# chu-tianxiang/QuIP-for-all

Hardware: AMD Instinct MI355X
Metric: decode tokens/sec bs=1 Llama-7B E8P12 2-bit, 1xMI355X; % HBM roofline (higher is better)
Workload: dtype i8xi8->i32 (fp16 I/O); 1 GPU; Llama-2-7B E8P12 random-init, bs=1 greedy decode, 1 hipGraph replay per token, positions [5, 833) of a 2048-slot static KV cache; layers=32, hidden=4096, ffn=11008, vocab=32000, parallelism=replicas x1 (no collective on the data path)

## Files before the change

include/quip_mi355.h:

```cpp
#ifndef QUIP_MI355_H_
#define QUIP_MI355_H_

#include <stddef.h>
#include <stdint.h>

#ifdef __cplusplus
extern "C" {
#endif

#define QUIP_ABI_VERSION 9

typedef void* quip_stream_t;

enum {
  QUIP_OK = 0,
  QUIP_ERR_NULL_POINTER = -1,
  QUIP_ERR_BAD_SHAPE = -2,
  QUIP_ERR_MISALIGNED = -3,
  QUIP_ERR_LAUNCH = -4,
  QUIP_ERR_UNSUPPORTED = -5,
  QUIP_NO_RESULT = 1
};

int quip_abi_version(void);
const char* quip_strerror(int code);
// ... 242 lines not shown
  const float* sin;
  const void* grid_packed_abs;
  void* workspace;
  void* dbg;
  int32_t n_layers, max_len, dbg_layer;
  float rms_eps, attn_scale;
  int32_t codebook;
  float resid_scale;
  int32_t shape;
  const void* grid2;
} quip_block_engine_args;
int quip_block_engine_supported(int32_t hidden, int32_t heads, int32_t kv_heads, int32_t head_dim, int32_t n_ffn, int32_t K);
size_t quip_block_engine_workspace_bytes(void);
size_t quip_block_engine_layer_bytes(void);
int quip_block_engine(const quip_block_engine_args* args, quip_stream_t stream);
int quip_debug_occupy(int32_t nwg, int32_t lds_bytes, int64_t ticks, void* sink, quip_stream_t stream);
int quip_block_engine_gqa_supported(int32_t hidden, int32_t heads, int32_t kv_heads, int32_t head_dim, int32_t n_ffn, int32_t K);
size_t quip_block_engine_gqa_workspace_bytes(void);
int quip_tile_codes(const void* qidxs, void* tiled, int64_t rows, int64_t row_bytes, quip_stream_t stream);
int quip_untile_codes(const void* tiled, void* qidxs, int64_t rows, int64_t row_bytes, quip_stream_t stream);
int quip_block_engine_g8_supported(int32_t hidden, int32_t heads, int32_t kv_heads, int32_t head_dim, int32_t n_ffn, int32_t K);
size_t quip_block_engine_g8_workspace_bytes(void);

#ifdef __cplusplus
}
#endif
#endif
```

quip_for_all_amd/capi.py:

```python
import ctypes
import os

_HERE = os.path.dirname(os.path.abspath(__file__))
LIB_PATH = os.environ.get("QUIP_LIB_PATH") or os.path.join(_HERE, "lib", "libquip_mi355.so")

_c = ctypes
_P, _I32, _I64, _F = _c.c_void_p, _c.c_int32, _c.c_int64, _c.c_float

SIGNATURES = {
    "quip_abi_version": [],
    "quip_device_cu_count": [],
    "quip_hadamard_f16": [_P, _P, _I64, _I32, _F, _P],
    "quip_hadamard": [_P, _P, _I64, _I32, _F, _I32, _P],
    "quip_had_transform_f16": [_P, _P, _I64, _I32, _I32, _I32, _I32, _P, _I32, _P, _P, _P, _P, _F, _P],
    "quip_had_transform_planes": [_P, _P, _I32, _I32, _I32, _P, _I32, _P, _F, _P],
    "quip_had_transform_fused_f16": [_P, _P, _I64, _I32, _I32, _I32, _I32, _P, _I32, _P, _P, _P, _P, _F, _P, _P],
    "quip_had_transform_planes_fused": [_P, _P, _I32, _I32, _I32, _P, _I32, _P, _F, _P, _P],
    "quip_had_transform_group_f16": [_P, _I32, _I64, _I32, _I32, _I32, _P],
    "quip_had_transform_planes_group": [_P, _I32, _I32, _I32, _I32, _P],
    "quip_e8p_gemv_planes_group": [_P, _P, _P, _P, _P, _I32, _I32, _P],
    "quip_e8p_gemv_workspace_bytes": [_I32],
    "quip_e8p_gemv_planes_ws": [_P, _P, _P, _P, _I32, _I32, _P, _c.c_size_t, _P],
    "quip_e8p_gemv_planes_group_ws": [_P, _P, _P, _P, _P, _I32, _I32, _P, _c.c_size_t, _P],
    "quip_had_transform_planes_rows": [_P, _I64, _I32, _I32, _I32, _P],
# ... 12 lines not shown
    "quip_rope_attn_workspace_bytes": [_I32, _I32],
    "quip_argmax_step_f16": [_P, _I32, _P, _P, _P],
    "quip_rope_attn_decode_f16": [_P, _P, _P, _P, _P, _P, _P, _P, _P, _I32, _I32, _I32, _I32, _F, _P, _P],
    "quip_rope_attn_decode_window_f16": [_P, _P, _P, _P, _P, _P, _P, _P, _P, _I32, _I32, _I32, _I32, _F, _I32, _P, _P],
    "quip_rope_attn_decode_z_window_f16": [_P, _P, _P, _P, _P, _P, _P, _P, _P, _I32, _I32, _I32, _I32, _F, _I32, _P, _P],
    "quip_rope_attn_decode_z_supported": [_I32, _I32, _I32],
    "quip_rope_attn_decode_z_f16": [_P, _P, _P, _P, _P, _P, _P, _P, _P, _I32, _I32, _I32, _I32, _F, _P, _P],
    "quip_rope_attn_batched_workspace_bytes": [_I32, _I32, _I32],
    "quip_rope_attn_decode_batched_f16": [_P, _P, _P, _P, _P, _P, _P, _P, _P, _I32, _I32, _I32, _I32, _I32, _F, _I32,
                                          _P, _P],
    "quip_argmax_step_batched_f16": [_P, _I32, _I32, _P, _P, _P],
    "quip_block_engine_supported": [_I32, _I32, _I32, _I32, _I32, _I32],
    "quip_block_engine_workspace_bytes": [],
    "quip_block_engine_layer_bytes": [],
    "quip_block_engine": [_P, _P],
    "quip_debug_occupy": [_I32, _I32, _c.c_int64, _P, _P],
    "quip_block_engine_gqa_supported": [_I32, _I32, _I32, _I32, _I32, _I32],
    "quip_block_engine_gqa_workspace_bytes": [],
    "quip_block_engine_g8_supported": [_I32, _I32, _I32, _I32, _I32, _I32],
    "quip_block_engine_g8_workspace_bytes": [],
    "quip_e8p_gemv_kernel_choice": [_P, _I32, _I32],
    "quip_ffn_engine_supported": [_I32, _I32, _I32],
    "quip_ffn_engine_workspace_bytes": [_I32, _I32],
    "quip_ffn_engine": [_P, _P],
    "quip_tile_codes": [_P, _P, _I64, _I64, _P],
    "quip_untile_codes": [_P, _P, _I64, _I64, _P],
    "quip_e8p_mm_origorder": [_P, _P, _P, _P, _I32, _I32, _I32, _P],
    "quip_e8p_mm_batched": [_P, _P, _P, _P, _I64, _I32, _I32, _P],
    "quip_e8prvq4_mm_batched": [_P, _P, _P, _F, _P, _I64, _I32, _I32, _P],
    "quip_e8prvq3_mm_batched": [_P, _P, _P, _P, _F, _P, _I64, _I32, _I32, _P],
# ... 47 lines not shown

class FfnEngineArgs(_c.Structure):
    _fields_ = [("w_gate", _P), ("w_up", _P), ("w_down", _P), ("planes_gate", _P), ("planes_up", _P), ("had3", _P),
                ("sv_gate", _P), ("sv_up", _P), ("su_down", _P), ("z_down", _P), ("grid_packed_abs", _P),
                ("workspace", _P), ("dbg", _P), ("out_scale", _F), ("in_scale", _F), ("hidden", _I32),
                ("n_ffn", _I32), ("K", _I32)]


class BlockEngineArgs(_c.Structure):
    _fields_ = [("layers", _P), ("h_in", _P), ("h_out", _P), ("pos", _P), ("cos", _P), ("sin", _P),
                ("grid_packed_abs", _P), ("workspace", _P), ("dbg", _P), ("n_layers", _I32), ("max_len", _I32),
                ("dbg_layer", _I32), ("rms_eps", _F), ("attn_scale", _F), ("codebook", _I32), ("resid_scale", _F),
                ("shape", _I32), ("grid2", _P)]


class HadFusion(_c.Structure):
    _fields_ = [("residual", _P), ("rms_weight", _P), ("gate", _P), ("rms_eps", _F)]


_lib = None


class QuipNativeError(RuntimeError):
    pass


def lib():
    global _lib
    if _lib is None:
        if not os.path.exists(LIB_PATH):
# ... 27 lines not shown
```

quip_for_all_amd/csrc/capi.hip:

```cpp
#include <stdlib.h>

#include <initializer_list>

#include "quip_internal.h"

namespace quip {

int device_cu_count() {
  static int cached[16] = {0};
  int dev = 0;
  if (hipGetDevice(&dev) != hipSuccess || dev < 0 || dev >= 16) return 256;
  if (cached[dev] == 0) {
    int v = 0;
    if (hipDeviceGetAttribute(&v, hipDeviceAttributeMultiprocessorCount, dev) != hipSuccess || v <= 0)
      v = 256;
    cached[dev] = v;
  }
  return cached[dev];
}

int device_cu_count_strict() {
  int dev = 0, v = 0;
  if (hipGetDevice(&dev) != hipSuccess) return 0;
  if (hipDeviceGetAttribute(&v, hipDeviceAttributeMultiprocessorCount, dev) != hipSuccess || v <= 0) return 0;
// ... 482 lines not shown
  if (in->n_layers < 1 || in->max_len < 1) return QUIP_ERR_BAD_SHAPE;
  BlockEngineArgs a;
  a.layers = in->layers; a.h_in = in->h_in; a.h_out = in->h_out; a.pos = in->pos; a.cos = in->cos; a.sin = in->sin;
  a.grid = in->grid_packed_abs; a.workspace = in->workspace; a.dbg = in->dbg;
  a.n_layers = in->n_layers; a.max_len = in->max_len; a.dbg_layer = in->dbg_layer;
  a.rms_eps = in->rms_eps; a.attn_scale = in->attn_scale; a.codebook = in->codebook; a.resid_scale = in->resid_scale;
  a.grid2 = in->grid2;
  if (in->codebook == 4 && (!in->grid2 || (reinterpret_cast<uintptr_t>(in->grid2) & 7u) != 0))
    return in->grid2 ? QUIP_ERR_MISALIGNED : QUIP_ERR_NULL_POINTER;
  if (in->shape == 1) return block_engine_gqa_launch(a, (hipStream_t)stream);
  if (in->shape == 2) return block_engine_g8_launch(a, (hipStream_t)stream);
  if (in->shape != 0) return QUIP_ERR_UNSUPPORTED;
  return block_engine_launch(a, (hipStream_t)stream);
}

namespace {
__global__ void tile_codes_kernel(const uint4* __restrict__ src, uint4* __restrict__ dst, long long pieces, int row_u4) {
  const long long i = (long long)blockIdx.x * blockDim.x + threadIdx.x;
  if (i >= pieces) return;
  const int n = (int)(i & 15), q = (int)((i >> 4) & 3);
  const long long cc = i >> 6;
  const int pieces_per_row = row_u4 / 4;
  const long long rb = cc / pieces_per_row;
  const int c = (int)(cc - rb * pieces_per_row);
  dst[i] = src[(rb * 16 + n) * row_u4 + c * 4 + q];
}
__global__ void untile_codes_kernel(const uint4* __restrict__ src, uint4* __restrict__ dst, long long pieces, int row_u4) {
  const long long i = (long long)blockIdx.x * blockDim.x + threadIdx.x;
  if (i >= pieces) return;
  const int n = (int)(i & 15), q = (int)((i >> 4) & 3);
// ... 429 lines not shown
```

quip_for_all_amd/csrc/decode_block.hip:

```cpp
#include "e8p_gemv_core.hip.h"
#include "engine_sync.hip.h"
#include "fht_wg512x.hip.h"

#ifndef QUIP_INO_EXACT
#define QUIP_INO_EXACT 0
#endif
#ifndef QUIP_PREDECODE_DOWN
#define QUIP_PREDECODE_DOWN 2
#endif
#ifndef QUIP_PREDECODE_QKV
#define QUIP_PREDECODE_QKV 2
#endif
#ifndef QUIP_QKV_ISSUE_EARLY
#define QUIP_QKV_ISSUE_EARLY 0
#endif
#ifndef QUIP_OWNER_PREDECODE
#define QUIP_OWNER_PREDECODE 1
#endif
#ifndef QUIP_ATT_STAMPS
#define QUIP_ATT_STAMPS 0
#endif
#if QUIP_ATT_STAMPS
#define ASTAMP(i) BSTAMP(18 + (i))
#else
// ... 46 lines not shown

struct BlockArgs {
  const BlockLayer* layers;
  const f16* h_in;
  f16* h_out;
  const int64_t* pos;
  const float* cos;
  const float* sin;
  const uint64_t* grid;
  char* ws;
  uint64_t* dbg;
  int n_layers, max_len, dbg_layer;
  float rms_eps, attn_scale;
  float resid_scale;
  const void* grid2;
};

constexpr int kWaves = 8, kThreads = 512;
constexpr int HID = 4096, NWG = 256, RPW = 16, HD = 128, NH = 32;
#ifndef QUIP_BLOCK_G8
#define QUIP_BLOCK_G8 0
#endif
constexpr bool G8 = QUIP_BLOCK_G8 != 0;
constexpr int NKVH = G8 ? 8 : NH, GQH = NH / NKVH;
constexpr int FK = G8 ? 56 : 43, FLOGL = 8, FL = 256, NFFN = FK * FL, FRB = 3;
constexpr int NGU = G8 ? 7 : 6;
constexpr int KPD = G8 ? 14336 : 11264, JD = G8 ? 28 : 22;
constexpr int ND = G8 ? 4 : 3;
constexpr float kMixScale = G8 ? 0.35355339059327373f : 1.f;
constexpr int QKB = G8 ? 384 : 768;
// ... 224 lines not shown
  };
#define SLOTS(m) std::integral_constant<unsigned, (m)>{}
  constexpr unsigned M_QKV = G8 ? 0x00cu : (RVQ ? 0x03fu : 0x007u), M_O = RVQ ? 0x0c0u : 0x008u, M_GATE = RVQ ? 0x03fu : 0x007u;
  constexpr unsigned M_UP = G8 ? 0x078u : (RVQ ? 0x1c0u : 0x038u) , M_DOWN = G8 ? 0x183u : (RVQ ? 0x03fu : 0x1c0u);
  static_assert(!G8 || (!RVQ && !HI && (REP == 24 || REP == 4)), "the grouped-query 4096-wide shape: E8P12 only");

  u32x2 tsrc;
  asm volatile("global_load_dwordx2 %0, %1, off" : "=v"(tsrc) : "v"(NIB ? table_source_ptr_nib(a.grid, lane, wave) : T::kD4 ? table_source_ptr_d4(a.grid, lane, wave) : table_source_ptr(a.grid, lane, wave)) : "memory");
  u32x2 tsrc3 = {0u, 0u};
  if constexpr (R3)
    asm volatile("global_load_dwordx2 %0, %1, off" : "=v"(tsrc3) : "v"(reinterpret_cast<const uint2*>(a.grid2) + (wave * 32 + (lane & 31))) : "memory");
  uint32_t gen;
  esync::ld4(gen, ctl);
  uint32_t hreg[4];
  uint32_t hraw[8];
#pragma unroll
  for (int k = 0; k < 8; ++k)
    asm volatile("global_load_ushort %0, %1, off" : "=v"(hraw[k]) : "v"(reinterpret_cast<const uint16_t*>(a.h_in) + tid + 512 * k) : "memory");
  {
    const BlockLayer& L0 = a.layers[0];
    if constexpr (RVQ) ISSUE_RVQ_QKV(L0); else if constexpr (G8) { ISSUE8_QKV(L0, 0); ISSUE8_QKV(L0, 1); } else { ISSUE(L0, 0); ISSUE(L0, 1); ISSUE(L0, 2); }
  }
  constexpr int NQ = RVQ ? 12 : (G8 ? 4 : 6);
  int* accs = reinterpret_cast<int*>(smem + B::kAcc);
  for (int i = tid; i < B::kAccRows * 4; i += kThreads) accs[i] = 0;
  asm volatile("s_waitcnt vmcnt(%2)" : "+v"(tsrc), "+v"(tsrc3) : "n"(9 + NQ) : "memory");
  if constexpr (NIB) fill_tables_nib(tsrc, lane, wave);
  else fill_tables_from_lane<REP>(smem, tsrc, lane, wave);
  fill_t3_from_lane<REP>(smem, tsrc3, lane, wave);
  asm volatile("s_waitcnt vmcnt(%1)" : "+v"(gen) : "n"(8 + NQ) : "memory");
  const uint32_t ebase = ((uint32_t)__builtin_amdgcn_readfirstlane((int)gen) + 1u) << 10;
  asm volatile("s_waitcnt vmcnt(%8)" : "+v"(hraw[0]), "+v"(hraw[1]), "+v"(hraw[2]), "+v"(hraw[3]), "+v"(hraw[4]), "+v"(hraw[5]),
               "+v"(hraw[6]), "+v"(hraw[7]) : "n"(NQ) : "memory");
// ... 1375 lines not shown
      for (int i = 0; i < NPQ; ++i) decode_pre(SQf(i), Bq[i]);
    }
    {
      const int c_lo = qc_lo, c_hi = qc_hi;
      edge(std::true_type{}, std::integral_constant<int, 2>{}, SLOTS(0u), 5, ebase | hop, 0x4000u, sv_d_prev, Ld.ln[0], Ld.su[c_lo], Ld.su[c_hi],
           Ld.sc[c_lo], Ld.sc[c_hi], c_hi != c_lo,
           [&]() { BSTAMP(1); if constexpr (RVQ) { ISSUE_RVQ_QKV_G(Ld, 0); ISSUE_RVQ_QKV_G(Ld, 1); } else if constexpr (!kPreQkv) { ISSUE(Ld, 0); ISSUE(Ld, 1); } },
           [&]() { if constexpr (RVQ) ISSUE_RVQ_QKV_G(Ld, 2); else if constexpr (!kPreQkv) ISSUE(Ld, 2); }, [&]() {}, 23,
           std::integral_constant<int, RVQ ? 8 : (kPreQkv ? 0 : 4)>{});
      BSTAMP(2);
    }
    if (more) P1_products(std::integral_constant<bool, kPreQkv>{}, Bq);
    esync::drain();
    own_slots(SLOTS(M_QKV));
  }
  if (w == 0) {
    uint32_t e, fp;
    esync::ld4(e, ctl + 1);
    esync::ld4(fp, ctl + 2);
    esync::drain();
    esync::own(e);
    esync::own(fp);
    const bool failed = __builtin_amdgcn_readfirstlane((int)e) != 0;
#pragma unroll
    for (int j = 0; j < 4; ++j) {
      reinterpret_cast<uint16_t*>(a.h_out)[tid + 512 * (2 * j)] = failed ? (uint16_t)0x7e00 : (uint16_t)(hreg[j] & 0xffffu);
      reinterpret_cast<uint16_t*>(a.h_out)[tid + 512 * (2 * j + 1)] = failed ? (uint16_t)0x7e00 : (uint16_t)(hreg[j] >> 16);
    }
    if (tid == 0) {
      if (failed && fp == 0u) esync::st_word(ctl + 2, (uint32_t)pos + 1u);
      esync::st_word(ctl, ebase >> 10);
      if (!failed && (ebase >> 10) >= (1u << 22) - 2u) esync::st_word(ctl + 1, 0xE000u);
    }
  }
#undef BSTAMP
#undef ISSUE
#undef SLOTS
#undef OFFC
#undef ISSUE_RVQ_QKV
#undef ISSUE_RVQ_O
#undef ISSUE_RVQ_GATE
#undef ISSUE_RVQ_UP_A
#undef ISSUE_RVQ_UP_B
#undef ISSUE_RVQ_GATE_G
#undef ISSUE_RVQ_DOWN_G0
#undef ISSUE_RVQ_QKV_G
#undef ISSUE_RVQ_DOWN_G1
#undef ISSUE_RVQ_DOWN_G2
#undef ISSUE_RVQ_UP_A_G
#undef ISSUE_RVQ_DOWN
}

}

#if QUIP_BLOCK_G8
size_t block_engine_g8_workspace_bytes() { return kWsBytes; }

bool block_engine_g8_supported(int hidden, int heads, int kv_heads, int head_dim, int n_ffn, int K) {
  return hidden == HID && heads == NH && kv_heads == NKVH && head_dim == HD && n_ffn == NFFN && K == 7 &&
         device_cu_count_strict() >= NWG;
}

int block_engine_g8_launch(const BlockEngineArgs& in, hipStream_t stream) {
  if (in.n_layers < 1 || in.n_layers > 146) return QUIP_ERR_BAD_SHAPE;
  if (in.codebook != 0) return QUIP_ERR_UNSUPPORTED;
  BlockArgs a;
  a.layers = reinterpret_cast<const BlockLayer*>(in.layers);
  a.h_in = reinterpret_cast<const f16*>(in.h_in);
  a.h_out = reinterpret_cast<f16*>(in.h_out);
  a.pos = reinterpret_cast<const int64_t*>(in.pos);
  a.cos = in.cos; a.sin = in.sin;
  a.grid = reinterpret_cast<const uint64_t*>(in.grid);
  a.ws = reinterpret_cast<char*>(in.workspace);
  a.dbg = reinterpret_cast<uint64_t*>(in.dbg);
  a.n_layers = in.n_layers; a.max_len = in.max_len; a.dbg_layer = in.dbg_layer;
  a.rms_eps = in.rms_eps; a.attn_scale = in.attn_scale; a.resid_scale = 0.f;
  a.grid2 = nullptr;
  static const bool rep24 = getenv("QUIP_ENG_REP") && atoi(getenv("QUIP_ENG_REP")) == 24;
  auto go = [&](auto kern, int lds, DynLdsCache& configured, ResidencyCache& resident) -> int {
    if (ensure_dyn_lds(configured, reinterpret_cast<const void*>(kern), lds) != QUIP_OK) return QUIP_ERR_LAUNCH;
    if (!persistent_grid_fits(resident, reinterpret_cast<const void*>(kern), kThreads, lds, NWG)) return QUIP_ERR_UNSUPPORTED;
    hipLaunchKernelGGL(kern, dim3(NWG), dim3(kThreads), lds, stream, a);
    return hipGetLastError() == hipSuccess ? QUIP_OK : QUIP_ERR_LAUNCH;
  };
  static DynLdsCache c24, c4;
  static ResidencyCache r24, r4;
  if (rep24) return go(decode_block_kernel<24>, BLds<24>::kBytes, c24, r24);
  return go(decode_block_kernel<4>, BLds<4>::kBytes, c4, r4);
}
#else
size_t block_engine_workspace_bytes() { return kWsBytes; }
size_t block_engine_layer_bytes() { return sizeof(BlockLayer); }
// ... 5 lines not shown

int block_engine_launch(const BlockEngineArgs& in, hipStream_t stream) {
  if (in.n_layers < 1 || in.n_layers > 146) return QUIP_ERR_BAD_SHAPE;
  BlockArgs a;
  a.layers = reinterpret_cast<const BlockLayer*>(in.layers);
  a.h_in = reinterpret_cast<const f16*>(in.h_in);
  a.h_out = reinterpret_cast<f16*>(in.h_out);
  a.pos = reinterpret_cast<const int64_t*>(in.pos);
  a.cos = in.cos; a.sin = in.sin;
  a.grid = reinterpret_cast<const uint64_t*>(in.grid);
  a.ws = reinterpret_cast<char*>(in.workspace);
  a.dbg = reinterpret_cast<uint64_t*>(in.dbg);
  a.n_layers = in.n_layers; a.max_len = in.max_len; a.dbg_layer = in.dbg_layer;
  a.rms_eps = in.rms_eps; a.attn_scale = in.attn_scale; a.resid_scale = 0.f;
  a.grid2 = in.grid2;
  auto go = [&](auto kern, int lds, DynLdsCache& configured, ResidencyCache& resident) -> int {
    if (ensure_dyn_lds(configured, reinterpret_cast<const void*>(kern), lds) != QUIP_OK) return QUIP_ERR_LAUNCH;
    if (!persistent_grid_fits(resident, reinterpret_cast<const void*>(kern), kThreads, lds, NWG)) return QUIP_ERR_UNSUPPORTED;
    hipLaunchKernelGGL(kern, dim3(NWG), dim3(kThreads), lds, stream, a);
    return hipGetLastError() == hipSuccess ? QUIP_OK : QUIP_ERR_LAUNCH;
  };
  static DynLdsCache c16, c64;
  static DynLdsCache crvq, chi, crvq3;
  static ResidencyCache r16, r24, r64, rrvq, rhi, rrvq3;
  if (in.codebook == 4) {
    if (!in.grid2) return QUIP_ERR_NULL_POINTER;
    a.resid_scale = in.resid_scale;
    return go(decode_block_kernel<12, true>, BLds<12, true>::kBytes, crvq3, rrvq3);
  }
  if (in.codebook == 3) return go(decode_block_kernel<64, true, true>, BLds<64, true>::kBytes, chi, rhi);
// ... 15 lines not shown
```

quip_for_all_amd/csrc/quip_internal.h:

```cpp
#pragma once
#include <hip/hip_runtime.h>
#include <stdint.h>

#include "../../include/quip_mi355.h"

namespace quip {

int device_cu_count();
struct ResidencyCache { signed char ok[16] = {}; };
bool persistent_grid_fits(ResidencyCache& cache, const void* kernel, int threads, int lds, int nwg);
int device_cu_count_strict();

struct DynLdsCache { int bytes[16] = {}; };
int ensure_dyn_lds(DynLdsCache& cache, const void* kernel, int lds);

struct GemvTune {
  int rep = 0;
  int rows = 0;
  int blocks = 0;
  int waves_g = 0;
  int max_waves = 0;
  int digits = 0;
  const void* grid2 = nullptr;
  void* dbg = nullptr;
// ... 151 lines not shown
struct BlockEngineArgs {
  const void* layers = nullptr;
  const void* h_in = nullptr;
  void* h_out = nullptr;
  const void* pos = nullptr;
  const float* cos = nullptr;
  const float* sin = nullptr;
  const void* grid = nullptr;
  void* workspace = nullptr;
  void* dbg = nullptr;
  int n_layers = 0, max_len = 0, dbg_layer = -1;
  float rms_eps = 1e-5f, attn_scale = 1.f;
  int codebook = 0;
  float resid_scale = 0.f;
  const void* grid2 = nullptr;
};
bool block_engine_supported(int hidden, int heads, int kv_heads, int head_dim, int n_ffn, int K);
size_t block_engine_workspace_bytes();
size_t block_engine_layer_bytes();
int block_engine_launch(const BlockEngineArgs& in, hipStream_t stream);
bool block_engine_gqa_supported(int hidden, int heads, int kv_heads, int head_dim, int n_ffn, int K);
size_t block_engine_gqa_workspace_bytes();
size_t block_engine_gqa_layer_bytes();
int block_engine_gqa_launch(const BlockEngineArgs& in, hipStream_t stream);
bool block_engine_g8_supported(int hidden, int heads, int kv_heads, int head_dim, int n_ffn, int K);
size_t block_engine_g8_workspace_bytes();
int block_engine_g8_launch(const BlockEngineArgs& in, hipStream_t stream);
int had_transform_planes_launch(const void* x, void* planes, int in_features, int n, int K,
                                const void* had, int transpose, const void* pre, float scale,
                                hipStream_t stream, const HadFusion* fuse = nullptr);
// ... 25 lines not shown
```

quip_for_all_amd/decode.py:

```python
import math
from dataclasses import dataclass

import torch
import torch.nn.functional as F

from .codebook import codebook_id
from .qlinear import (QuantLinear, chain_planes, chain_supported, ffn_engine, ffn_engine_ok, forward_group,
                      fused_in_supported, gemv_chain, gemv_fused, gemv_group_unfused, gemv_unfused, out_transform_group)


@dataclass
class LlamaShape:
    hidden: int = 4096
    ffn: int = 11008
    layers: int = 32
    heads: int = 32
    kv_heads: int = 32
    vocab: int = 32000
    rms_eps: float = 1e-5
    rope_theta: float = 10000.0

    @property
    def head_dim(self):
        return self.hidden // self.heads
# ... 197 lines not shown
        planes_ok = all(hasattr(m.codebook, "mm_planes") and m.codebook.planes_supported(m.q_out_features, m.q_in_features)
                        for m in L0.values() if isinstance(m, QuantLinear))
        self.chain = (planes_ok and os.environ.get("QUIP_CHAIN", "1") != "0"
                      and chain_supported(qkv0, L0["down"]) and chain_supported(gu0, L0["o"]))
        prologue_ok = (planes_ok and fused_in_supported(qkv0, prev=L0["down"]) and fused_in_supported(gu0, prev=L0["o"]))
        self.o_fused = planes_ok and fused_in_supported([L0["o"]])
        self.qkv_fused = planes_ok and fused_in_supported(qkv0)
        self.fused_prologue = os.environ.get("QUIP_FUSED_PROLOGUE", "1") != "0" and (self.chain or prologue_ok)
        self.ffn_eng = (self.fused_prologue and self.chain and os.environ.get("QUIP_FFN_ENGINE", "1") != "0"
                        and all(ffn_engine_ok(L["gate"], L["up"], L["down"]) for L in self.layers))
        self.ffn_ws = None
        if self.ffn_eng:
            from .register_lib import ffn_engine_workspace
            self.ffn_ws = ffn_engine_workspace(s.ffn, L0["gate"].K_right, self.dev)
        self.block_eng = False
        d4 = all(getattr(m.codebook, "id", None) in ("D4", "E8P12RVQ4B", "HI", "E8P12RVQ3B") for m in L0.values() if isinstance(m, QuantLinear))
        gqa_shape = self.fused_prologue and self.chain and s.kv_heads != s.heads and s.hidden in (8192, 4096)
        if ((self.ffn_eng or gqa_shape or (d4 and self.fused_prologue and self.chain and os.environ.get("QUIP_FFN_ENGINE", "1") != "0"))
                and os.environ.get("QUIP_BLOCK_ENGINE", "1") != "0" and not self.window):
            self._init_block_engine()
        from .register_lib import rope_attn_decode_z_supported
        self.attn_z = (self.fused_prologue and self.fused_attention and os.environ.get("QUIP_ATTN_Z", "1") != "0"
                       and rope_attn_decode_z_supported(s.heads, s.kv_heads, s.head_dim)
                       and all(l.K_right == 1 and not l.per_channel and l.bias is None and l.SV is not None
                               and l.q_out_features == l.out_features == (s.heads if i == 0 else s.kv_heads) * s.head_dim
                               for i, l in enumerate(qkv0)))

    def _init_block_engine(self):
        import numpy as np
        from .qlinear import _engine_had3
# ... 196 lines not shown
    def _attention(self, i, q, k, v, cos, sin, mask):
        s = self.s
        if self.fused_attention:
            return torch.ops.quip_lib.rope_attn_decode(
                q.view(s.heads, s.head_dim), k.view(s.kv_heads, s.head_dim), v.view(s.kv_heads, s.head_dim),
                self.cos, self.sin, self.pos, self.kcache[i], self.vcache[i], self.attn_ws, self.window)
        q = self._rope(q.view(1, s.heads, 1, s.head_dim), cos, sin)
        k = self._rope(k.view(1, s.kv_heads, 1, s.head_dim), cos, sin)
        self.kcache[i].index_copy_(1, self.pos, k[0])
        self.vcache[i].index_copy_(1, self.pos, v.view(s.kv_heads, 1, s.head_dim))
        return F.scaled_dot_product_attention(q, self.kcache[i][None], self.vcache[i][None], attn_mask=mask,
                                              enable_gqa=(s.kv_heads != s.heads))

    def step(self):
        s = self.s
        h = self.embed[self.tok]
        cos = sin = mask = None
        if not self.fused_attention:
            cos, sin = self.cos[self.pos], self.sin[self.pos]
            mask = (self.arange[None, None, None, :] <= self.pos)
            if self.window:
                mask = mask & (self.arange[None, None, None, :] > self.pos - self.window)
        if getattr(self, "block_eng", False):
            h = torch.ops.quip_lib.block_engine(self.eng_layers, h.reshape(-1), self.pos, self.cos, self.sin,
                                                self.eng_grid, self.eng_ws, len(self.layers), self.max_len, s.rms_eps,
                                                1.0 / math.sqrt(s.head_dim), None, -1, self.eng_codebook, self.eng_resid_scale,
                                                getattr(self, "eng_shape", 0), getattr(self, "eng_grid2", None),
                                                *((self.kcache, self.vcache) if torch.is_tensor(self.kcache) else (None, None)))
            return self._head(h.reshape(1, -1))
        if self.fused_prologue:
            return self._step_fused(h, cos, sin, mask)
        for i, L in enumerate(self.layers):
            self._rm_enter(L)
            q, k, v = forward_group([L["q"], L["k"], L["v"]], h, rms_weight=L["ln1"], rms_eps=s.rms_eps)
            a = self._attention(i, q, k, v, cos, sin, mask)
            h = L["o"].forward_fused(a.reshape(1, s.hidden), residual=h)
            g, u = forward_group([L["gate"], L["up"]], h, rms_weight=L["ln2"], rms_eps=s.rms_eps)
            h = L["down"].forward_fused(u, gate=g, residual=h)
            self._rm_exit(L)
        return self._head(h)

    def _step_fused(self, h, cos, sin, mask):
        s = self.s
        zd = prev_down = None
        for i, L in enumerate(self.layers):
            self._rm_enter(L)
            qkv = [L["q"], L["k"], L["v"]]
            if zd is None and self.qkv_fused:
                _, zs = gemv_fused(qkv, x=h, rms_weight=L["ln1"], rms_eps=s.rms_eps)
            elif zd is None:
                zs = gemv_group_unfused(qkv, h, rms_weight=L["ln1"], rms_eps=s.rms_eps)
            else:
                h, zs = self._zx(qkv, prev_down, zd, h, L["ln1"])
            if self.attn_z:
                a = torch.ops.quip_lib.rope_attn_decode_z(
# ... 202 lines not shown
```

quip_for_all_amd/hf_fast.py:

```python
import torch

from . import register_lib as _R

_HANDLES = {}
import os as _os
_ASSUME_UNPADDED = _os.environ.get("QUIP_FAST_DECODE_ASSUME_UNPADDED", "0") != "0"
_PREFILL = _os.environ.get("QUIP_FAST_DECODE_PREFILL", "1") != "0"
try:
    _R._lib.define("hf_decode_step(Tensor input_ids, Tensor(a!)[] keys, Tensor(b!)[] values, Tensor(c!)[] lens, int handle) -> Tensor")
except RuntimeError:
    pass


def _wrapper_of(handle):
    fd = _HANDLES.get(handle, lambda: None)()
    if fd is None:
        raise RuntimeError("quip_lib::hf_decode_step: the model this compiled graph was traced for no longer exists")
    return fd


def _hf_decode_step_cuda(input_ids, keys, values, lens, handle):
    return _wrapper_of(handle)._static_step(input_ids, keys, values, lens)


# ... 155 lines not shown
    def _step_checked(self, dec, set_inputs):
        set_inputs()
        logits = dec.step()
        if (getattr(dec, "block_eng", False) or getattr(dec, "ffn_eng", False)) and not torch.cuda.is_current_stream_capturing():
            st = dec.engine_status()
            if st:
                dec.engine_reset()
                if st != 0xE000:
                    import warnings
                    warnings.warn("persistent decode launch gave up on a hand-off (code 0x%x): the device was shared with "
                                  "other work; fast decode continues on the stage-wise step" % st)
                    dec.block_eng = dec.ffn_eng = False
                    dec.graph = None
                set_inputs()
                logits = dec.step()
        return logits

    def _dynamic_decoder(self, dev):
        from .decode import LlamaDecoder
        if self.dyn is None or self.dyn.dev != dev:
            try:
                self.dyn = _off_thread(lambda: LlamaDecoder.from_hf(self.model, max_len=self._dyn_capacity(),
                                                                    assume_llama_like=self.assume_llama_like))
            except (NotImplementedError, TypeError, ValueError) as e:
                self.disabled = repr(e)
                return None
            self.dyn_owner = None
        return self.dyn

    def _release_owner(self, cache):
# ... 153 lines not shown
```

Baseline: 845.0 tokens/s.

## Fuse embedding lookup, final norm, LM head and argmax into persistent block engine

Extends the persistent block-engine kernel so one launch covers a whole token. It reads the embedding row for the current token on device, runs all layers, then applies the final RMSNorm, the fp16 LM-head GEMV split across the 256 workgroups, and a cross-workgroup argmax that writes the next token and position. This removes the separate embedding gather, head and argmax launches, and the gaps between them, from each graph replay. In exchange it adds a grid-wide handshake at the tail and extra code paths, and it requires hidden=4096 with fp16 embed and head weights.

```diff
diff --git a/include/quip_mi355.h b/include/quip_mi355.h
--- a/include/quip_mi355.h
+++ b/include/quip_mi355.h
@@ -8,7 +8,7 @@
 extern "C" {
 #endif
 
-#define QUIP_ABI_VERSION 9
+#define QUIP_ABI_VERSION 10
 
 typedef void* quip_stream_t;
 
@@ -281,6 +281,17 @@
 size_t quip_block_engine_workspace_bytes(void);
 size_t quip_block_engine_layer_bytes(void);
 int quip_block_engine(const quip_block_engine_args* args, quip_stream_t stream);
+typedef struct quip_token_tail_args {
+  void* tok;
+  void* pos;
+  const void* embed;
+  const void* final_norm;
+  const void* lm_head;
+  void* logits;
+  void* xnorm;
+  int32_t vocab;
+} quip_token_tail_args;
+int quip_block_engine_token(const quip_block_engine_args* args, const quip_token_tail_args* tail, quip_stream_t stream);
 int quip_debug_occupy(int32_t nwg, int32_t lds_bytes, int64_t ticks, void* sink, quip_stream_t stream);
 int quip_block_engine_gqa_supported(int32_t hidden, int32_t heads, int32_t kv_heads, int32_t head_dim, int32_t n_ffn, int32_t K);
 size_t quip_block_engine_gqa_workspace_bytes(void);
diff --git a/quip_for_all_amd/capi.py b/quip_for_all_amd/capi.py
--- a/quip_for_all_amd/capi.py
+++ b/quip_for_all_amd/capi.py
@@ -50,6 +50,7 @@
     "quip_block_engine_workspace_bytes": [],
     "quip_block_engine_layer_bytes": [],
     "quip_block_engine": [_P, _P],
+    "quip_block_engine_token": [_P, _P, _P],
     "quip_debug_occupy": [_I32, _I32, _c.c_int64, _P, _P],
     "quip_block_engine_gqa_supported": [_I32, _I32, _I32, _I32, _I32, _I32],
     "quip_block_engine_gqa_workspace_bytes": [],
@@ -127,6 +128,11 @@
                 ("shape", _I32), ("grid2", _P)]
 
 
+class TokenTailArgs(_c.Structure):
+    _fields_ = [("tok", _P), ("pos", _P), ("embed", _P), ("final_norm", _P), ("lm_head", _P), ("logits", _P),
+                ("xnorm", _P), ("vocab", _I32)]
+
+
 class HadFusion(_c.Structure):
     _fields_ = [("residual", _P), ("rms_weight", _P), ("gate", _P), ("rms_eps", _F)]
 
diff --git a/quip_for_all_amd/csrc/capi.hip b/quip_for_all_amd/csrc/capi.hip
--- a/quip_for_all_amd/csrc/capi.hip
+++ b/quip_for_all_amd/csrc/capi.hip
@@ -520,6 +520,33 @@
   return block_engine_launch(a, (hipStream_t)stream);
 }
 
+int quip_block_engine_token(const quip_block_engine_args* in, const quip_token_tail_args* t, quip_stream_t stream) {
+  if (!in || !t) return QUIP_ERR_NULL_POINTER;
+  if (!in->layers || !in->pos || !in->cos || !in->sin || !in->grid_packed_abs || !in->workspace || !t->tok || !t->pos ||
+      !t->embed || !t->final_norm || !t->lm_head || !t->logits)
+    return QUIP_ERR_NULL_POINTER;
+  if (!aligned16(in->layers) || !aligned16(in->workspace) || (in->h_out && !aligned16(in->h_out)) ||
+      (reinterpret_cast<uintptr_t>(in->grid_packed_abs) & 63u) != 0 || !aligned16(t->embed) || !aligned16(t->lm_head) ||
+      !aligned16(t->logits) || !aligned16(t->final_norm) || (t->xnorm && !aligned16(t->xnorm)) ||
+      (reinterpret_cast<uintptr_t>(t->tok) & 7u) != 0 || (reinterpret_cast<uintptr_t>(t->pos) & 7u) != 0)
+    return QUIP_ERR_MISALIGNED;
+  if (in->n_layers < 1 || in->max_len < 1 || t->vocab < 256 || t->vocab >= 256 * 65535) return QUIP_ERR_BAD_SHAPE;
+  if (t->pos != in->pos) return QUIP_ERR_BAD_SHAPE;
+  if (in->shape != 0 && in->shape != 2) return QUIP_ERR_UNSUPPORTED;
+  BlockEngineArgs a;
+  a.layers = in->layers; a.h_in = nullptr; a.h_out = in->h_out; a.pos = in->pos; a.cos = in->cos; a.sin = in->sin;
+  a.grid = in->grid_packed_abs; a.workspace = in->workspace; a.dbg = in->dbg;
+  a.n_layers = in->n_layers; a.max_len = in->max_len; a.dbg_layer = in->dbg_layer;
+  a.rms_eps = in->rms_eps; a.attn_scale = in->attn_scale; a.codebook = in->codebook; a.resid_scale = in->resid_scale;
+  a.grid2 = in->grid2;
+  if (in->codebook == 4 && (!in->grid2 || (reinterpret_cast<uintptr_t>(in->grid2) & 7u) != 0))
+    return in->grid2 ? QUIP_ERR_MISALIGNED : QUIP_ERR_NULL_POINTER;
+  a.tok = t->tok; a.embed = t->embed; a.final_norm = t->final_norm; a.lm_head = t->lm_head; a.logits = t->logits;
+  a.xnorm = t->xnorm; a.vocab = t->vocab;
+  if (in->shape == 2) return block_engine_g8_launch(a, (hipStream_t)stream);
+  return block_engine_launch(a, (hipStream_t)stream);
+}
+
 namespace {
 __global__ void tile_codes_kernel(const uint4* __restrict__ src, uint4* __restrict__ dst, long long pieces, int row_u4) {
   const long long i = (long long)blockIdx.x * blockDim.x + threadIdx.x;
diff --git a/quip_for_all_amd/csrc/decode_block.hip b/quip_for_all_amd/csrc/decode_block.hip
--- a/quip_for_all_amd/csrc/decode_block.hip
+++ b/quip_for_all_amd/csrc/decode_block.hip
@@ -1,6 +1,7 @@
 #include "e8p_gemv_core.hip.h"
 #include "engine_sync.hip.h"
 #include "fht_wg512x.hip.h"
+#include "token_tail.hip.h"
 
 #ifndef QUIP_INO_EXACT
 #define QUIP_INO_EXACT 0
@@ -84,6 +85,7 @@
   float rms_eps, attn_scale;
   float resid_scale;
   const void* grid2;
+  tail::Args tail;
 };
 
 constexpr int kWaves = 8, kThreads = 512;
@@ -338,9 +340,15 @@
   esync::ld4(gen, ctl);
   uint32_t hreg[4];
   uint32_t hraw[8];
+  const bool whole_token = a.tail.lm_head != nullptr;
+  const f16* h_in = a.h_in;
+  if (whole_token) {
+    const long long tk = *a.tail.tok;
+    h_in = a.tail.embed + (size_t)(tk >= 0 && tk < (long long)a.tail.vocab ? tk : 0) * HID;
+  }
 #pragma unroll
   for (int k = 0; k < 8; ++k)
-    asm volatile("global_load_ushort %0, %1, off" : "=v"(hraw[k]) : "v"(reinterpret_cast<const uint16_t*>(a.h_in) + tid + 512 * k) : "memory");
+    asm volatile("global_load_ushort %0, %1, off" : "=v"(hraw[k]) : "v"(reinterpret_cast<const uint16_t*>(h_in) + tid + 512 * k) : "memory");
   {
     const BlockLayer& L0 = a.layers[0];
     if constexpr (RVQ) ISSUE_RVQ_QKV(L0); else if constexpr (G8) { ISSUE8_QKV(L0, 0); ISSUE8_QKV(L0, 1); } else { ISSUE(L0, 0); ISSUE(L0, 1); ISSUE(L0, 2); }
@@ -1746,6 +1754,12 @@
     esync::drain();
     own_slots(SLOTS(M_QKV));
   }
+  if (whole_token) {
+    static_assert(B::kArea % 16 == 0 && B::kAreaBytes >= tail::kLdsBytes, "the tail's x and reduction slots in the transient area");
+    const bool tst = a.dbg != nullptr && (a.dbg_layer & 0xffff) == a.n_layers;
+    ++hop;
+    tail::run(a.tail, hreg, smem + B::kArea, ctl, zbufs, ebase | hop, w, a.rms_eps, pos64, tst ? a.dbg + w * 32 : nullptr, dbg_rt);
+  }
   if (w == 0) {
     uint32_t e, fp;
     esync::ld4(e, ctl + 1);
@@ -1754,10 +1768,12 @@
     esync::own(e);
     esync::own(fp);
     const bool failed = __builtin_amdgcn_readfirstlane((int)e) != 0;
-#pragma unroll
-    for (int j = 0; j < 4; ++j) {
-      reinterpret_cast<uint16_t*>(a.h_out)[tid + 512 * (2 * j)] = failed ? (uint16_t)0x7e00 : (uint16_t)(hreg[j] & 0xffffu);
-      reinterpret_cast<uint16_t*>(a.h_out)[tid + 512 * (2 * j + 1)] = failed ? (uint16_t)0x7e00 : (uint16_t)(hreg[j] >> 16);
+    if (a.h_out) {
+#pragma unroll
+      for (int j = 0; j < 4; ++j) {
+        reinterpret_cast<uint16_t*>(a.h_out)[tid + 512 * (2 * j)] = failed ? (uint16_t)0x7e00 : (uint16_t)(hreg[j] & 0xffffu);
+        reinterpret_cast<uint16_t*>(a.h_out)[tid + 512 * (2 * j + 1)] = failed ? (uint16_t)0x7e00 : (uint16_t)(hreg[j] >> 16);
+      }
     }
     if (tid == 0) {
       if (failed && fp == 0u) esync::st_word(ctl + 2, (uint32_t)pos + 1u);
@@ -1783,6 +1799,20 @@
 #undef ISSUE_RVQ_DOWN
 }
 
+tail::Args tail_args(const BlockEngineArgs& in) {
+  tail::Args t;
+  if (!in.lm_head) return t;
+  t.tok = reinterpret_cast<int64_t*>(in.tok);
+  t.pos = reinterpret_cast<int64_t*>(const_cast<void*>(in.pos));
+  t.embed = reinterpret_cast<const f16*>(in.embed);
+  t.norm_w = reinterpret_cast<const f16*>(in.final_norm);
+  t.lm_head = reinterpret_cast<const f16*>(in.lm_head);
+  t.logits = reinterpret_cast<f16*>(in.logits);
+  t.xnorm = reinterpret_cast<f16*>(in.xnorm);
+  t.vocab = in.vocab;
+  return t;
+}
+
 }
 
 #if QUIP_BLOCK_G8
@@ -1808,6 +1838,7 @@
   a.n_layers = in.n_layers; a.max_len = in.max_len; a.dbg_layer = in.dbg_layer;
   a.rms_eps = in.rms_eps; a.attn_scale = in.attn_scale; a.resid_scale = 0.f;
   a.grid2 = nullptr;
+  a.tail = tail_args(in);
   static const bool rep24 = getenv("QUIP_ENG_REP") && atoi(getenv("QUIP_ENG_REP")) == 24;
   auto go = [&](auto kern, int lds, DynLdsCache& configured, ResidencyCache& resident) -> int {
     if (ensure_dyn_lds(configured, reinterpret_cast<const void*>(kern), lds) != QUIP_OK) return QUIP_ERR_LAUNCH;
@@ -1843,6 +1874,7 @@
   a.n_layers = in.n_layers; a.max_len = in.max_len; a.dbg_layer = in.dbg_layer;
   a.rms_eps = in.rms_eps; a.attn_scale = in.attn_scale; a.resid_scale = 0.f;
   a.grid2 = in.grid2;
+  a.tail = tail_args(in);
   auto go = [&](auto kern, int lds, DynLdsCache& configured, ResidencyCache& resident) -> int {
     if (ensure_dyn_lds(configured, reinterpret_cast<const void*>(kern), lds) != QUIP_OK) return QUIP_ERR_LAUNCH;
     if (!persistent_grid_fits(resident, reinterpret_cast<const void*>(kern), kThreads, lds, NWG)) return QUIP_ERR_UNSUPPORTED;
diff --git a/quip_for_all_amd/csrc/quip_internal.h b/quip_for_all_amd/csrc/quip_internal.h
--- a/quip_for_all_amd/csrc/quip_internal.h
+++ b/quip_for_all_amd/csrc/quip_internal.h
@@ -189,6 +189,13 @@
   int codebook = 0;
   float resid_scale = 0.f;
   const void* grid2 = nullptr;
+  void* tok = nullptr;
+  const void* embed = nullptr;
+  const void* final_norm = nullptr;
+  const void* lm_head = nullptr;
+  void* logits = nullptr;
+  void* xnorm = nullptr;
+  int vocab = 0;
 };
 bool block_engine_supported(int hidden, int heads, int kv_heads, int head_dim, int n_ffn, int K);
 size_t block_engine_workspace_bytes();
diff --git a/quip_for_all_amd/csrc/token_tail.hip.h b/quip_for_all_amd/csrc/token_tail.hip.h
--- /dev/null
+++ b/quip_for_all_amd/csrc/token_tail.hip.h
@@ -0,0 +1,198 @@
+#pragma once
+#include <limits.h>
+
+#include "engine_sync.hip.h"
+#include "quip_device.hip.h"
+
+namespace quip {
+namespace tail {
+
+struct Args {
+  int64_t* tok = nullptr;
+  int64_t* pos = nullptr;
+  const f16* embed = nullptr;
+  const f16* norm_w = nullptr;
+  const f16* lm_head = nullptr;
+  f16* logits = nullptr;
+  f16* xnorm = nullptr;
+  int vocab = 0;
+};
+
+constexpr int kHid = 4096, kWgs = 256, kWvs = 8, kThr = 512;
+constexpr int kRowU4 = kHid / 8;
+constexpr int kRoundingChain = 8 * 2 + 2 + 6;
+constexpr int kLdsBytes = kHid * 2 + 256;
+constexpr uint32_t kGiveUpCode = 0x9000u;
+
+__device__ __forceinline__ bool better(float v, int i, float best, int bi) { return v > best || (v == best && i < bi); }
+
+__device__ __forceinline__ void st_half_device(f16* p, uint16_t bits) {
+  asm volatile("global_store_short %0, %1, off sc1" : : "v"(p), "v"((uint32_t)bits) : "memory");
+}
+
+__device__ __forceinline__ void row_range(int vocab, int w, int& row0, int& nrows) {
+  const int q = vocab >> 8, r = vocab & 255;
+  row0 = w * q + (w < r ? w : r);
+  nrows = q + (w < r ? 1 : 0);
+}
+
+__device__ __forceinline__ float dot_row(const u32x4 (&W)[8], const u32x4 (&x)[8]) {
+  float a0 = 0.f, a1 = 0.f, a2 = 0.f, a3 = 0.f;
+#pragma unroll
+  for (int i = 0; i < 8; ++i) {
+    a0 = __builtin_amdgcn_fdot2(as_f16x2(W[i].x), as_f16x2(x[i].x), a0, false);
+    a1 = __builtin_amdgcn_fdot2(as_f16x2(W[i].y), as_f16x2(x[i].y), a1, false);
+    a2 = __builtin_amdgcn_fdot2(as_f16x2(W[i].z), as_f16x2(x[i].z), a2, false);
+    a3 = __builtin_amdgcn_fdot2(as_f16x2(W[i].w), as_f16x2(x[i].w), a3, false);
+  }
+  return (a0 + a1) + (a2 + a3);
+}
+
+__device__ __forceinline__ void run(const Args& t, const uint32_t (&hreg)[4], char* lds, uint32_t* ctl, uint64_t* gran,
+                                    uint32_t tag, int w, float eps, long long pos64, uint64_t* stamps, bool stamps_rt) {
+  const int tid = threadIdx.x, lane = tid & 63;
+  const int wave = __builtin_amdgcn_readfirstlane(tid >> 6);
+#define TSTAMP(i) do { if (stamps && tid == 0) stamps[i] = stamps_rt ? __builtin_amdgcn_s_memrealtime() : __builtin_amdgcn_s_memtime(); } while (0)
+  TSTAMP(0);
+  f16* xs = reinterpret_cast<f16*>(lds);
+  double* redd = reinterpret_cast<double*>(lds + kHid * 2);
+  float* redv = reinterpret_cast<float*>(lds + kHid * 2 + 64);
+  int* redi = reinterpret_cast<int*>(lds + kHid * 2 + 96);
+
+  uint32_t err;
+  esync::ld4(err, ctl + 1);
+  uint16_t wn[8];
+#pragma unroll
+  for (int k = 0; k < 8; ++k) wn[k] = reinterpret_cast<const uint16_t*>(t.norm_w)[tid + 512 * k];
+  esync::drain();
+  esync::own(err);
+  const bool failed = __builtin_amdgcn_readfirstlane((int)err) != 0;
+
+  float h[8];
+#pragma unroll
+  for (int j = 0; j < 4; ++j) {
+    const f16x2 hh = as_f16x2(hreg[j]);
+    h[2 * j] = (float)hh.x;
+    h[2 * j + 1] = (float)hh.y;
+  }
+  double ss = 0.0;
+#pragma unroll
+  for (int k = 0; k < 8; ++k) ss = __builtin_fma((double)h[k], (double)h[k], ss);
+#pragma unroll
+  for (int o = 32; o >= 1; o >>= 1) ss += __shfl_xor(ss, o, 64);
+  __builtin_amdgcn_s_barrier();
+  if (lane == 0) redd[wave] = ss;
+  asm volatile("s_waitcnt lgkmcnt(0)\n\ts_barrier" ::: "memory");
+  double tot = 0.0;
+#pragma unroll
+  for (int i = 0; i < kWvs; ++i) tot += redd[i];
+  const float rs = (float)(1.0 / __builtin_sqrt(tot * (1.0 / kHid) + (double)eps));
+  {
+#pragma clang fp contract(off)
+#pragma unroll
+    for (int k = 0; k < 8; ++k) {
+      const f16 xk = (f16)((h[k] * rs) * (float)__builtin_bit_cast(f16, wn[k]));
+      xs[tid + 512 * k] = xk;
+      if (t.xnorm && w == 0) t.xnorm[tid + 512 * k] = xk;
+    }
+  }
+  asm volatile("s_waitcnt lgkmcnt(0)\n\ts_barrier" ::: "memory");
+  u32x4 x[8];
+#pragma unroll
+  for (int i = 0; i < 8; ++i) x[i] = reinterpret_cast<const u32x4*>(lds)[64 * i + lane];
+  TSTAMP(1);
+
+  int row0, nrows;
+  row_range(t.vocab, w, row0, nrows);
+  const u32x4* Wm = reinterpret_cast<const u32x4*>(t.lm_head) + (size_t)row0 * kRowU4 + lane;
+  auto request = [&](int lr, u32x4 (&d)[8]) {
+    const u32x4* p = Wm + (size_t)lr * kRowU4;
+#pragma unroll
+    for (int i = 0; i < 8; ++i) d[i] = __builtin_nontemporal_load(p + 64 * i);
+  };
+  float best = -3.0e38f;
+  int bi = INT_MAX;
+  auto finish = [&](int lr, float s) {
+#pragma unroll
+    for (int o = 32; o >= 1; o >>= 1) s += __shfl_xor(s, o, 64);
+    s = __builtin_bit_cast(float, __builtin_amdgcn_readfirstlane(__builtin_bit_cast(int, s)));
+    const f16 hv = failed ? __builtin_bit_cast(f16, (uint16_t)0x7e00) : (f16)s;
+    if (lane == 0) st_half_device(t.logits + row0 + lr, __builtin_bit_cast(uint16_t, hv));
+    const float v = (float)hv;
+    if (better(v, lr, best, bi)) { best = v; bi = lr; }
+  };
+  u32x4 A[8], Bw[8];
+  if (wave < nrows) request(wave, A);
+  if (wave + kWvs < nrows) request(wave + kWvs, Bw);
+  for (int lr = wave; lr < nrows; lr += 2 * kWvs) {
+    const float sa = dot_row(A, x);
+    if (lr + 2 * kWvs < nrows) request(lr + 2 * kWvs, A);
+    finish(lr, sa);
+    if (lr + kWvs < nrows) {
+      const float sb = dot_row(Bw, x);
+      if (lr + 3 * kWvs < nrows) request(lr + 3 * kWvs, Bw);
+      finish(lr + kWvs, sb);
+    }
+  }
+  TSTAMP(2);
+
+  esync::drain();
+  if (lane == 0) { redv[wave] = best; redi[wave] = bi; }
+  asm volatile("s_waitcnt lgkmcnt(0)\n\ts_barrier" ::: "memory");
+  if (wave == 0) {
+    best = redv[0]; bi = redi[0];
+#pragma unroll
+    for (int i = 1; i < kWvs; ++i)
+      if (better(redv[i], redi[i], best, bi)) { best = redv[i]; bi = redi[i]; }
+    const uint32_t word = ((uint32_t)__builtin_bit_cast(uint16_t, (f16)best) << 16) | (bi == INT_MAX ? 0xffffu : (uint32_t)bi);
+    if (lane == 0) esync::st_granule(gran + w, word, tag);
+  }
+  TSTAMP(3);
+  if (w != 0) return;
+
+  asm volatile("s_barrier" ::: "memory");
+  if (wave < 4) {
+    esync::u32x2_t g;
+    uint32_t spins = 0;
+    for (;;) {
+      esync::ld8(g, gran + tid);
+      esync::drain();
+      esync::own(g);
+      if (esync::spin_step(g.y == tag, spins, ctl + 1, kGiveUpCode)) break;
+    }
+    int r0, nr;
+    row_range(t.vocab, tid, r0, nr);
+    const bool have = g.y == tag && (g.x & 0xffffu) != 0xffffu;
+    float v = have ? (float)__builtin_bit_cast(f16, (uint16_t)(g.x >> 16)) : -3.0e38f;
+    int idx = have ? r0 + (int)(g.x & 0xffffu) : INT_MAX;
+#pragma unroll
+    for (int o = 32; o >= 1; o >>= 1) {
+      const float ov = __shfl_xor(v, o, 64);
+      const int oi = __shfl_xor(idx, o, 64);
+      if (better(ov, oi, v, idx)) { v = ov; idx = oi; }
+    }
+    if (lane == 0) { redv[wave] = v; redi[wave] = idx; }
+  }
+  asm volatile("s_waitcnt lgkmcnt(0)\n\ts_barrier" ::: "memory");
+  best = redv[0]; bi = redi[0];
+#pragma unroll
+  for (int i = 1; i < 4; ++i)
+    if (better(redv[i], redi[i], best, bi)) { best = redv[i]; bi = redi[i]; }
+  uint32_t err2;
+  esync::ld4(err2, ctl + 1);
+  esync::drain();
+  esync::own(err2);
+  const bool failed2 = __builtin_amdgcn_readfirstlane((int)err2) != 0;
+  if (failed2 && !failed) {
+    for (int i = tid; i < t.vocab; i += kThr) st_half_device(t.logits + i, (uint16_t)0x7e00);
+  }
+  if (tid == 0) {
+    *t.tok = (!failed2 && bi < t.vocab) ? (int64_t)bi : (int64_t)0;
+    *t.pos = (int64_t)pos64 + 1;
+  }
+  TSTAMP(4);
+#undef TSTAMP
+}
+
+}
+}
diff --git a/quip_for_all_amd/decode.py b/quip_for_all_amd/decode.py
--- a/quip_for_all_amd/decode.py
+++ b/quip_for_all_amd/decode.py
@@ -4,6 +4,7 @@
 import torch
 import torch.nn.functional as F
 
+from . import token_tail as _token_tail
 from .codebook import codebook_id
 from .qlinear import (QuantLinear, chain_planes, chain_supported, ffn_engine, ffn_engine_ok, forward_group,
                       fused_in_supported, gemv_chain, gemv_fused, gemv_group_unfused, gemv_unfused, out_transform_group)
@@ -235,6 +236,7 @@
             from .register_lib import ffn_engine_workspace
             self.ffn_ws = ffn_engine_workspace(s.ffn, L0["gate"].K_right, self.dev)
         self.block_eng = False
+        self.token_tail = os.environ.get("QUIP_TOKEN_TAIL", "1") != "0"
         d4 = all(getattr(m.codebook, "id", None) in ("D4", "E8P12RVQ4B", "HI", "E8P12RVQ3B") for m in L0.values() if isinstance(m, QuantLinear))
         gqa_shape = self.fused_prologue and self.chain and s.kv_heads != s.heads and s.hidden in (8192, 4096)
         if ((self.ffn_eng or gqa_shape or (d4 and self.fused_prologue and self.chain and os.environ.get("QUIP_FFN_ENGINE", "1") != "0"))
@@ -461,6 +463,17 @@
 
     def step(self):
         s = self.s
+        if self._token_tail_on():
+            lg = self.__dict__.get("_tail_logits")
+            if lg is None or lg.shape[1] != self.lm_head.shape[0] or lg.device != self.lm_head.device:
+                lg = self._tail_logits = torch.empty(1, self.lm_head.shape[0], dtype=torch.float16, device=self.lm_head.device)
+            torch.ops.quip_lib.block_engine_token(self.eng_layers, self.tok, self.pos, self.embed, self.final_norm, self.lm_head,
+                                                  lg, self.cos, self.sin, self.eng_grid, self.eng_ws, len(self.layers),
+                                                  self.max_len, s.rms_eps, 1.0 / math.sqrt(s.head_dim), None, -1,
+                                                  self.eng_codebook, self.eng_resid_scale, self.eng_shape,
+                                                  getattr(self, "eng_grid2", None),
+                                                  *((self.kcache, self.vcache) if torch.is_tensor(self.kcache) else (None, None)))
+            return lg
         h = self.embed[self.tok]
         cos = sin = mask = None
         if not self.fused_attention:
@@ -486,6 +499,16 @@
             h = L["down"].forward_fused(u, gate=g, residual=h)
             self._rm_exit(L)
         return self._head(h)
+
+    def _token_tail_on(self):
+        if not (getattr(self, "block_eng", False) and getattr(self, "token_tail", True)
+                and getattr(self, "sampling", None) is None and getattr(self, "eng_shape", 0) in (0, 2)):
+            return False
+        lm, em = self.lm_head, self.embed
+        return (lm.is_cuda and lm.dtype == torch.float16 and lm.is_contiguous() and lm.dim() == 2 and lm.shape[1] == 4096
+                and 256 <= lm.shape[0] < 256 * 65535 and em.dtype == torch.float16 and em.is_contiguous()
+                and em.shape == lm.shape and em.device == lm.device and self.final_norm.dtype == torch.float16
+                and self.final_norm.is_contiguous() and len(self.layers) <= 146)
 
     def _step_fused(self, h, cos, sin, mask):
         s = self.s
diff --git a/quip_for_all_amd/hf_fast.py b/quip_for_all_amd/hf_fast.py
--- a/quip_for_all_amd/hf_fast.py
+++ b/quip_for_all_amd/hf_fast.py
@@ -193,6 +193,8 @@
                     dec.graph = None
                 set_inputs()
                 logits = dec.step()
+        if logits is dec.__dict__.get("_tail_logits"):
+            logits = logits.clone()
         return logits
 
     def _dynamic_decoder(self, dev):
diff --git a/quip_for_all_amd/token_tail.py b/quip_for_all_amd/token_tail.py
--- /dev/null
+++ b/quip_for_all_amd/token_tail.py
@@ -0,0 +1,72 @@
+import ctypes
+
+import torch
+
+from . import capi
+from . import register_lib as _R
+
+try:
+    _R._lib.define("block_engine_token(Tensor layers, Tensor(a!) tok, Tensor(b!) pos, Tensor embed, Tensor final_norm, "
+                   "Tensor lm_head, Tensor(c!) logits, Tensor cos, Tensor sin, Tensor grid, Tensor(d!) workspace, "
+                   "int n_layers, int max_len, float rms_eps, float attn_scale, Tensor? dbg=None, int dbg_layer=-1, "
+                   "int codebook=0, float resid_scale=0.0, int shape=0, Tensor? grid2=None, "
+                   "Tensor(e!)? kcache=None, Tensor(f!)? vcache=None, Tensor(g!)? xnorm=None) -> ()")
+except RuntimeError:
+    pass
+
+
+def _block_engine_token_cuda(layers, tok, pos, embed, final_norm, lm_head, logits, cos, sin, grid, workspace, n_layers,
+                             max_len, rms_eps, attn_scale, dbg=None, dbg_layer=-1, codebook=0, resid_scale=0.0, shape=0,
+                             grid2=None, kcache=None, vcache=None, xnorm=None):
+    need = _R._need
+    dev = lm_head.device
+    lb = capi.lib().quip_block_engine_layer_bytes()
+    need(layers.dtype == torch.uint8 and layers.is_contiguous() and layers.numel() >= n_layers * lb and layers.device == dev,
+         "layers must be the packed descriptors (uint8, n_layers x 256 bytes) on the device")
+    need(shape in (0, 2), "block_engine_token: shape 0 (hidden 4096, multi-head) or 2 (hidden 4096, grouped-query)")
+    for t in (tok, pos):
+        need(t.dtype == torch.int64 and t.numel() == 1 and t.device == dev, "tok / pos: int64 device scalars")
+    need(lm_head.dtype == torch.float16 and lm_head.is_contiguous() and lm_head.dim() == 2 and lm_head.shape[1] == 4096,
+         "lm_head: contiguous fp16 (vocab, 4096)")
+    vocab = lm_head.shape[0]
+    need(embed.dtype == torch.float16 and embed.is_contiguous() and tuple(embed.shape) == (vocab, 4096) and embed.device == dev,
+         "embed: contiguous fp16 (vocab, 4096) on lm_head's device")
+    need(final_norm.dtype == torch.float16 and final_norm.is_contiguous() and final_norm.numel() == 4096
+         and final_norm.device == dev, "final_norm: fp16 [4096]")
+    need(logits.dtype == torch.float16 and logits.is_contiguous() and logits.numel() == vocab and logits.device == dev,
+         "logits: contiguous fp16 with vocab elements")
+    if xnorm is not None:
+        need(xnorm.dtype == torch.float16 and xnorm.is_contiguous() and xnorm.numel() == 4096 and xnorm.device == dev,
+             "xnorm: fp16 [4096]")
+    for t in (cos, sin):
+        need(t.dtype == torch.float32 and t.is_contiguous() and t.shape == (max_len, 128) and t.device == dev,
+             "cos / sin: fp32 [max_len, 128]")
+    need(workspace.dtype == torch.uint8 and workspace.device == dev and workspace.numel() >= _R._block_engine_ws_bytes(shape),
+         "workspace too small")
+    if codebook in (1, 3):
+        g = _R._d4_grid_f16(grid)
+        need(g.device == dev and g.numel() == 1024, "D4 / HI grid: fp16 (256, 4) on the device")
+    else:
+        g = _R._grid_i64(grid, lm_head)
+    if codebook == 4:
+        need(grid2 is not None and grid2.dtype == torch.int8 and grid2.is_contiguous() and grid2.numel() == 2048
+             and grid2.device == dev, "grid2: the E81B table as int8 (256, 8) on the device")
+    a = capi.BlockEngineArgs(layers.data_ptr(), None, None, pos.data_ptr(), cos.data_ptr(), sin.data_ptr(), g.data_ptr(),
+                             workspace.data_ptr(), _R._ptr(dbg), int(n_layers), int(max_len), int(dbg_layer), float(rms_eps),
+                             float(attn_scale), int(codebook), float(resid_scale), int(shape),
+                             _R._ptr(grid2) if codebook == 4 else None)
+    t = capi.TokenTailArgs(tok.data_ptr(), pos.data_ptr(), embed.data_ptr(), final_norm.data_ptr(), lm_head.data_ptr(),
+                           logits.data_ptr(), _R._ptr(xnorm), int(vocab))
+    with torch.cuda.device(dev):
+        capi.check(capi.lib().quip_block_engine_token(ctypes.byref(a), ctypes.byref(t), _R._stream(lm_head)),
+                   "quip_block_engine_token")
+
+
+try:
+    _R._lib.impl("block_engine_token", _block_engine_token_cuda, "CUDA")
+    _R._reg_fake("block_engine_token",
+                 lambda layers, tok, pos, embed, final_norm, lm_head, logits, cos, sin, grid, workspace, n_layers, max_len,
+                 rms_eps, attn_scale, dbg=None, dbg_layer=-1, codebook=0, resid_scale=0.0, shape=0, grid2=None, kcache=None,
+                 vcache=None, xnorm=None: None)
+except RuntimeError:
+    pass
```

Measured after the change: 878.3 tokens/s (median of 6 runs). 3.9% higher.
